# nlesc-dirac/sagecal

Hardware: NVIDIA H100
Metric: baseline_visibilities_per_sec_predict_jacobian (higher is better)
Workload: dtype f64

## Files before the change

sagecal_b200/csrc/internal.cuh:

```cuda
#pragma once
#include <cuda_runtime.h>
#include <stdint.h>
#include <stdio.h>
#include <stdlib.h>

#define DB_CHECK(call)                                                                          \
  do {                                                                                          \
    cudaError_t err__ = (call);                                                                 \
    if (err__ != cudaSuccess) {                                                                 \
      fprintf(stderr, "dirac_b200: CUDA error %s at %s:%d: %s\n", cudaGetErrorName(err__),      \
              __FILE__, __LINE__, cudaGetErrorString(err__));                                   \
      exit(1);          \
    }                                                                                           \
  } while (0)


#define TILE_P 8
#define TILE_Q 32
#define TILE_THREADS (TILE_P * TILE_Q)

struct TileDesc {
  short pb, qb;
};

// ... 250 lines not shown
  const double *mu_dev;
  double mu;
  int lower;
  int N, Nbase;
};

enum { DB_OPT_CP_ROWS = 0, DB_OPT_LINE_DIRECT = 1, DB_OPT_OS_CONSISTENT = 2,
       DB_OPT_RTR_NU_UNJOINED = 3, DB_OPT_ADMM_LM = 4, DB_OPT_SWEEP_RESIDUAL = 5,
       DB_OPT_COUNT = 8 };
int db_opt(int id);
int db_sm_count();
static inline int db_cp_max_slices(int Nbase, int tilesz) {
  const int nbg = (Nbase + 255) / 256;
  int nsl = (db_sm_count() + nbg - 1) / nbg;
  if ((tilesz + 31) / 32 > nsl) nsl = (tilesz + 31) / 32;
  return nsl;
}

extern "C" {
void db_launch_coh_to_planar(const double2 *src, double2 *dst, long long r0, int nr, int M,
                             long long R, cudaStream_t st);
void db_launch_coh_from_planar(const double2 *src, double2 *dst, long long r0, int nr, int M,
                               long long R, cudaStream_t st);
void db_launch_vis_to_planar(const double2 *src, double2 *dst, long long R, cudaStream_t st);
void db_launch_vis_from_planar(const double2 *src, double2 *dst, long long R, cudaStream_t st);
void db_launch_grad_tma(const GradArgs *a, int ntile, cudaStream_t st);
void db_launch_grad_window_tma(const GradArgs *a, int ntile, long long r_lo, long long r_hi,
                               cudaStream_t st);
void db_launch_grad_band_tma(const GradArgs *a, int ntile, int nchan, cudaStream_t st);
int db_cluster_pass_nblocks(int ntile, int nt, int tslice);
enum { DB_CP_LIN = 0, DB_CP_LIN_GRAD = 1, DB_CP_SPLIT = 2, DB_CP_TILE = 3, DB_CP_NONE = 4 };
int db_launch_cluster_pass(const ClusterPassArgs *a, int ntile, cudaStream_t st);
int db_cluster_pass_forms_hidden(int N, int Nbase);
void db_launch_coh_gram(const GramArgs *a, int ntile, int nk, cudaStream_t st);
void db_launch_station_sums(const AssembleArgs *a, int nb, cudaStream_t st);
void db_launch_assemble_tiles(const AssembleArgs *a, int nb, cudaStream_t st);
void db_launch_batch_mu0(const double *Hst, double *mu, int N, double tau, int nb, cudaStream_t st);
void db_launch_copy_add_diag(const double *A0, double *A, int n, double mu, cudaStream_t st);
int db_chol_max_n();
int db_chol_available();
size_t db_chol_ws_doubles(int n);
int db_tri_available(int n);
void db_chol_set_step(const double *pcur, double *pnew, double *sc, double *zero);
void db_launch_tri_solve(const double *L, int n, const double *b, double *x, cudaStream_t st);
void db_launch_tri_solve_ld(const double *L, int ld, int n, const double *b, double *x,
                            cudaStream_t st);
void db_launch_chol_factor_batched(const double *A, int n, const double *mu, double *ws,
                                   long long ws_stride, int *info, int nb, cudaStream_t st);
void db_launch_chol_solve(const double *A, int n, double mu, const double *b, double *x, double *ws,
                          int *info, cudaStream_t st);
int db_bigtri_available(int n);
size_t db_bigtri_ws_doubles(int n);
void db_launch_bigtri_solve(const double *L, int ld, int n, const double *b, double *x, double *ws,
                            unsigned epoch, int invert, cudaStream_t st);
int db_stream_all_nblocks(int Nbase, int tilesz);
void db_launch_predict_tma(const StreamAllArgs *a, cudaStream_t st);
void db_launch_cost_window_tma(const StreamAllArgs *a, cudaStream_t st);
int db_band_nblocks(int Nbase, int tilesz, int nchan);
void db_launch_band_tma(const StreamAllArgs *a, int nchan, cudaStream_t st);
void db_launch_band_tma(const StreamAllArgs *a, int nchan, cudaStream_t st);
unsigned db_launch_line_setup_tma(const StreamAllArgs *a, cudaStream_t st);
void db_launch_line_poly_finish(const double *part, unsigned nparts, double *partials, double *out,
                                unsigned int *counter, cudaStream_t st);
void db_line_setup_shape_reset();
void db_line_setup_shape(int *shape);
}
```

sagecal_b200/csrc/kernels_bigtri.cu:

```cuda
#include "internal.cuh"

#define BT 64
#define BT_THREADS 256
#define BT_PENDING 0x7ff8dead0badbeefull

__device__ __forceinline__ unsigned ld_acquire(const unsigned *p) {
  unsigned v;
  asm volatile("ld.acquire.gpu.u32 %0, [%1];" : "=r"(v) : "l"(p) : "memory");
  return v;
}
__device__ __forceinline__ void st_release(unsigned *p, unsigned v) {
  asm volatile("st.release.gpu.u32 [%0], %1;" ::"l"(p), "r"(v) : "memory");
}

__global__ void __launch_bounds__(BT)
k_bigtri_diag_inv(const double *__restrict__ L, int ld, double *__restrict__ Linv) {
  __shared__ double Ls[BT * BT];
  const int blk = blockIdx.x, c = threadIdx.x;
  const double *src = L + (size_t)(blk * BT) * ld + blk * BT;
  for (int e = threadIdx.x; e < BT * BT; e += BT) {
    const int cc = e / BT, r = e % BT;
    Ls[cc * BT + r] = (r >= cc) ? src[(size_t)cc * ld + r] : 0.0;
  }
  __syncthreads();
  double x[BT];
#pragma unroll
  for (int r = 0; r < BT; r++) x[r] = 0.0;
#pragma unroll
  for (int r = 0; r < BT; r++) {
    double s = (r == c) ? 1.0 : 0.0;
#pragma unroll
    for (int k = 0; k < BT; k++)
      if (k < r) s = fma(-Ls[k * BT + r], x[k], s);
    x[r] = (r >= c) ? s / Ls[r * BT + r] : 0.0;
  }
  double *dst = Linv + (size_t)blk * BT * BT + (size_t)c * BT;
#pragma unroll
  for (int r = 0; r < BT; r++) dst[r] = x[r];
}

struct BigTriArgs {
  const double *L;
  const double *Linv;
  const double *rhs;
  double *out;
  unsigned *flags;
  unsigned epoch;
  int n, ld, nb;
};

template <bool FWD>
__global__ void __launch_bounds__(BT_THREADS)
k_bigtri(BigTriArgs a) {
  extern __shared__ __align__(16) double sm[];
  double *Lc = sm;
  double *Li = Lc + BT * BT;
  double *vec = Li + BT * BT;
  double *part = vec + BT;
  const int tid = threadIdx.x, r = tid & (BT - 1), q = tid >> 6;
  const int me = FWD ? (int)blockIdx.x : a.nb - 1 - (int)blockIdx.x;
  const int nprev = FWD ? me : a.nb - 1 - me;
  {
    const double *inv = a.Linv + (size_t)me * BT * BT;
    for (int e = tid; e < BT * BT; e += BT_THREADS) {
      const int cc = e / BT, rr = e % BT;
      if (FWD) Li[cc * BT + rr] = inv[e];
      else Li[rr * BT + cc] = inv[e];
    }
    if (nprev > 0) {
      const int bi = FWD ? me : me + 1, bk = FWD ? me - 1 : me;
      const double *src = a.L + (size_t)(bk * BT) * a.ld + bi * BT;
      for (int e = tid; e < BT * BT; e += BT_THREADS) {
        const int cc = e / BT, rr = e % BT;
        const double v = src[(size_t)cc * a.ld + rr];
        if (FWD) Lc[cc * BT + rr] = v;
        else Lc[rr * BT + cc] = v;
      }
    }
  }
  double acc = 0.0;
  double nx[16];
  auto fetch = [&](int step) {
    const int other = FWD ? step : a.nb - 1 - step;
    if (FWD) {
      const double *src = a.L + (size_t)(other * BT + 16 * q) * a.ld + me * BT + r;
#pragma unroll
      for (int c = 0; c < 16; c++) nx[c] = __ldcg(src + (size_t)c * a.ld);
    } else {
      const double *src = a.L + (size_t)(me * BT + r) * a.ld + other * BT + 16 * q;
#pragma unroll
      for (int c = 0; c < 16; c++) nx[c] = __ldcg(src + c);
    }
  };
  const int noff = nprev > 0 ? nprev - 1 : 0;
  if (noff > 0) fetch(0);
  __syncthreads();
  for (int step = 0; step < nprev; step++) {
    const int other = FWD ? step : a.nb - 1 - step;
    if (tid < BT) {
      const unsigned long long *src = reinterpret_cast<const unsigned long long *>(a.out) +
                                      (size_t)other * BT + tid;
      unsigned long long bits;
      do {
        asm volatile("ld.relaxed.gpu.u64 %0, [%1];" : "=l"(bits) : "l"(src) : "memory");
      } while (bits == BT_PENDING);
      vec[tid] = __longlong_as_double((long long)bits);
    }
    __syncthreads();
    if (step < noff) {
      double cur[16];
#pragma unroll
      for (int c = 0; c < 16; c++) cur[c] = nx[c];
      if (step + 1 < noff) fetch(step + 1);
#pragma unroll
      for (int c = 0; c < 16; c++) acc = fma(-cur[c], vec[16 * q + c], acc);
    } else {
#pragma unroll
      for (int c = 0; c < 16; c++) acc = fma(-Lc[(16 * q + c) * BT + r], vec[16 * q + c], acc);
    }
    __syncthreads();
  }
  part[q * BT + r] = acc;
  __syncthreads();
  if (tid < BT)
    vec[tid] = a.rhs[(size_t)me * BT + tid] + part[tid] + part[BT + tid] + part[2 * BT + tid] +
               part[3 * BT + tid];
  __syncthreads();
  double s = 0.0;
#pragma unroll
  for (int c = 0; c < 16; c++) s = fma(Li[(16 * q + c) * BT + r], vec[16 * q + c], s);
  __syncthreads();
  part[q * BT + r] = s;
  __syncthreads();
  if (tid < BT) {
    const double v = part[tid] + part[BT + tid] + part[2 * BT + tid] + part[3 * BT + tid];
    asm volatile("st.relaxed.gpu.f64 [%0], %1;" ::"l"(a.out + (size_t)me * BT + tid), "d"(v) : "memory");
  }
}

__global__ void k_bigtri_arm(unsigned long long *y, unsigned long long *x, int n) {
  const int i = blockIdx.x * blockDim.x + threadIdx.x;
  if (i < n) {
    y[i] = BT_PENDING;
    x[i] = BT_PENDING;
  }
}

extern "C" {
int db_bigtri_available(int n) {
  if (getenv("DIRAC_B200_NO_BIGTRI")) return 0;
  return n > 512 && (n % BT) == 0 && n / BT <= db_sm_count();
}
size_t db_bigtri_ws_doubles(int n) { return (size_t)(n / BT) * BT * BT + (size_t)n + (size_t)(n / BT) + 16; }

void db_launch_bigtri_solve(const double *L, int ld, int n, const double *b, double *x, double *ws,
                            unsigned epoch, int invert, cudaStream_t st) {
  const int nb = n / BT;
  double *Linv = ws, *y = ws + (size_t)nb * BT * BT;
  unsigned *flags = reinterpret_cast<unsigned *>(y + n);
  static bool configured = false;
  const size_t smem = sizeof(double) * (2 * BT * BT + BT + 4 * BT);
  if (!configured) {
    DB_CHECK(cudaFuncSetAttribute(k_bigtri<true>, cudaFuncAttributeMaxDynamicSharedMemorySize, (int)smem));
    DB_CHECK(cudaFuncSetAttribute(k_bigtri<false>, cudaFuncAttributeMaxDynamicSharedMemorySize, (int)smem));
    configured = true;
  }
  if (invert) k_bigtri_diag_inv<<<nb, BT, 0, st>>>(L, ld, Linv);
  k_bigtri_arm<<<(n + 255) / 256, 256, 0, st>>>(reinterpret_cast<unsigned long long *>(y),
                                               reinterpret_cast<unsigned long long *>(x), n);
  BigTriArgs a;
  a.L = L; a.Linv = Linv; a.n = n; a.ld = ld; a.nb = nb;
  a.rhs = b; a.out = y; a.flags = flags; a.epoch = 2 * epoch + 1;
  k_bigtri<true><<<nb, BT_THREADS, smem, st>>>(a);
  a.rhs = y; a.out = x; a.flags = flags + nb; a.epoch = 2 * epoch + 2;
  k_bigtri<false><<<nb, BT_THREADS, smem, st>>>(a);
}

int dirac_b200_bigtri_solve(int n, const double *L, const double *b, double *x, int reps, double *us) {
  if (!db_bigtri_available(n)) return -1;
  double *dL, *db, *dx, *ws;
  const size_t nd = db_bigtri_ws_doubles(n);
  DB_CHECK(cudaMalloc((void **)&dL, sizeof(double) * (size_t)n * n));
  DB_CHECK(cudaMalloc((void **)&db, sizeof(double) * n));
  DB_CHECK(cudaMalloc((void **)&dx, sizeof(double) * n));
  DB_CHECK(cudaMalloc((void **)&ws, sizeof(double) * nd));
  DB_CHECK(cudaMemset(ws, 0, sizeof(double) * nd));
  DB_CHECK(cudaMemcpy(dL, L, sizeof(double) * (size_t)n * n, cudaMemcpyHostToDevice));
  DB_CHECK(cudaMemcpy(db, b, sizeof(double) * n, cudaMemcpyHostToDevice));
  unsigned epoch = 0;
  db_launch_bigtri_solve(dL, n, n, db, dx, ws, ++epoch, 1, 0);
  DB_CHECK(cudaDeviceSynchronize());
  DB_CHECK(cudaMemcpy(x, dx, sizeof(double) * n, cudaMemcpyDeviceToHost));
  if (reps > 0 && us) {
    cudaEvent_t e0, e1;
    DB_CHECK(cudaEventCreate(&e0));
    DB_CHECK(cudaEventCreate(&e1));
    DB_CHECK(cudaEventRecord(e0, 0));
    for (int i = 0; i < reps; i++) db_launch_bigtri_solve(dL, n, n, db, dx, ws, ++epoch, 0, 0);
    DB_CHECK(cudaEventRecord(e1, 0));
    DB_CHECK(cudaEventSynchronize(e1));
    float ms = 0.f;
    DB_CHECK(cudaEventElapsedTime(&ms, e0, e1));
    *us = 1e3 * ms / reps;
    cudaEventDestroy(e0);
    cudaEventDestroy(e1);
  }
  DB_CHECK(cudaGetLastError());
  cudaFree(dL); cudaFree(db); cudaFree(dx); cudaFree(ws);
  return 0;
}
}
```

sagecal_b200/csrc/lm.cu:

```cuda
#include <float.h>
#include <math.h>
#include <string.h>
#include <vector>

#include "../../include/dirac_b200.h"
#include "problem.h"

#define CS_CHECK(call)                                                                     \
  do {                                                                                     \
    cusolverStatus_t s__ = (call);                                                         \
    if (s__ != CUSOLVER_STATUS_SUCCESS) {                                                  \
      fprintf(stderr, "dirac_b200: cuSOLVER error %d at %s:%d\n", (int)s__, __FILE__, __LINE__); \
      exit(1);                                                                             \
    }                                                                                      \
  } while (0)
#define CB_CHECK(call)                                                                     \
  do {                                                                                     \
    cublasStatus_t s__ = (call);                                                           \
    if (s__ != CUBLAS_STATUS_SUCCESS) {                                                    \
      fprintf(stderr, "dirac_b200: cuBLAS error %d at %s:%d\n", (int)s__, __FILE__, __LINE__); \
      exit(1);                                                                             \
    }                                                                                      \
  } while (0)

// ... 30 lines not shown
  w.Tsub = dalloc<double>((size_t)d.Nbase * 16);
  w.JTJ0 = dalloc<double>((size_t)n8 * n8);
  w.JTJ = dalloc<double>((size_t)n8 * n8);
  w.JTe = d.scal + 64 + n8;
  w.JTe_new = d.scal + 64 + 2 * n8;
  w.Hst = dalloc<double>((size_t)4 * d.N);
  w.Dp = d.scal + 64;
  w.pnew = dalloc<double>(n8);
  w.plast = dalloc<double>(n8);
  w.pold = dalloc<double>(n8);
  w.devinfo = reinterpret_cast<int *>(d.scal + 64 + 3 * n8);
  w.tau = dalloc<double>(n8);
  w.svdS = w.svdU = w.svdVT = nullptr;
  w.wbuf = w.ebuf = nullptr;
  w.os_eps = w.os_w = nullptr;
  w.HP = w.HQ = nullptr;
  w.JB = w.LB = nullptr;
  w.sys_T = w.sys_p = w.sys_H = nullptr;
  w.pref_slot = (int *)malloc(sizeof(int) * d.M);
  for (int k = 0; k < d.M; k++) w.pref_slot[k] = -1;
  w.jtj0_cur = nullptr;
  w.jtj_spec = nullptr;
  {
    const int nbg = (d.Nbase + 255) / 256;
    const int nsl = db_cp_max_slices(d.Nbase, d.tilesz);
    w.jte_part = dalloc<double>((size_t)nbg * (nsl + 1) * n8);
  }
  DB_CHECK(cudaEventCreateWithFlags(&w.ev_mail, cudaEventDisableTiming));
  DB_CHECK(cudaMallocHost((void **)&w.h_vec, sizeof(double) * (5 * n8 + 4 * d.N + 64)));
  static cusolverDnHandle_t g_cs = nullptr;
  static cublasHandle_t g_cb = nullptr;
  if (!g_cs) {
    CS_CHECK(cusolverDnCreate(&g_cs));
    CB_CHECK(cublasCreate(&g_cb));
  }
  w.cs = g_cs;
  w.cb = g_cb;
  CS_CHECK(cusolverDnSetStream(w.cs, d.stream));
  CB_CHECK(cublasSetStream(w.cb, d.stream));
  int l1 = 0, l2 = 0, l3 = 0;
  CS_CHECK(cusolverDnDpotrf_bufferSize(w.cs, CUBLAS_FILL_MODE_LOWER, n8, w.JTJ, n8, &l1));
  CS_CHECK(cusolverDnDgeqrf_bufferSize(w.cs, n8, n8, w.JTJ, n8, &l2));
  CS_CHECK(cusolverDnDormqr_bufferSize(w.cs, CUBLAS_SIDE_LEFT, CUBLAS_OP_T, n8, 1, n8, w.JTJ, n8,
                                       w.tau, w.Dp, n8, &l3));
  w.lwork = l1 > l2 ? l1 : l2;
  if (l3 > w.lwork) w.lwork = l3;
  int l4 = 0;
  CS_CHECK(cusolverDnDgesvd_bufferSize(w.cs, n8, n8, &l4));
  if (l4 > w.lwork) w.lwork = l4;
  w.own_chol = n8 <= db_chol_max_n() && db_chol_available() && !getenv("DIRAC_B200_CUSOLVER");
  if (w.own_chol && (size_t)w.lwork < db_chol_ws_doubles(n8)) w.lwork = (int)db_chol_ws_doubles(n8);
  w.cswork = dalloc<double>((size_t)w.lwork);
  w.bc = (!w.own_chol && n8 > 1024) ? db_bigchol_create(n8, BC_BLOCK, BC_INV_PANEL, BC_LOOKAHEAD) : nullptr;
  w.bt_ws = nullptr;
  w.bt_epoch = 0;
  if (!w.own_chol && db_bigtri_available(n8)) {
    const size_t nd = db_bigtri_ws_doubles(n8);
    w.bt_ws = dalloc<double>(nd);
    DB_CHECK(cudaMemsetAsync(w.bt_ws, 0, sizeof(double) * nd, d.stream));
  }
  w.dbuf = dalloc<double2>((size_t)4 * d.R);
  w.ready = true;
}

static void robust_init(dirac_b200_problem *pr) {
  LMWork &w = pr->lm;
  if (w.wbuf) return;
  DevProblem &d = pr->d;
  w.wbuf = dalloc<double2>((size_t)4 * d.R);
  w.ebuf = dalloc<double2>((size_t)4 * d.R);
  w.HP = dalloc<double>((size_t)d.N * 20);
  w.HQ = dalloc<double>((size_t)d.N * 20);
}

static void os_init(dirac_b200_problem *pr) {
  robust_init(pr);
  LMWork &w = pr->lm;
  if (w.os_eps) return;
  w.os_eps = dalloc<double2>((size_t)4 * pr->d.R);
  w.os_w = dalloc<double2>((size_t)4 * pr->d.R);
}

void db_lm_free(dirac_b200_problem *pr) {
  LMWork &w = pr->lm;
  if (!w.ready) return;
  db_free(w.T); db_free(w.Tsub); db_free(w.JTJ0); db_free(w.JTJ);
  db_free(w.Hst); db_free(w.pnew); db_free(w.plast); db_free(w.pold); db_free(w.jte_part);
  db_free(w.tau); db_free(w.cswork); db_free(w.dbuf);
  if (w.bt_ws) db_free(w.bt_ws);
  db_bigchol_destroy(w.bc);
  if (w.svdS) { db_free(w.svdS); db_free(w.svdU); db_free(w.svdVT); }
  if (w.wbuf) { db_free(w.wbuf); db_free(w.ebuf); db_free(w.HP); db_free(w.HQ); }
  if (w.os_eps) { db_free(w.os_eps); db_free(w.os_w); }
  if (w.LB) {
    if (w.JB) db_free(w.JB);
    db_free(w.LB); db_free(w.HB); db_free(w.mu_dev); db_free(w.binfo_dev);
    db_free(w.LBptr_dev); db_free(w.blist_dev); db_free(w.btix_dev); db_free(w.bpoff_dev);
    cudaFreeHost(w.h_mu); cudaFreeHost(w.h_binfo);
  }
  free(w.pref_slot);
  cudaEventDestroy(w.ev_mail);
  cudaFreeHost(w.h_vec);
  free(w.T_valid);
  w.ready = false;
}

static int pick_tslice(const DevProblem &d, int nt) {
  int target_ctas = db_sm_count();
  int slices = (target_ctas + d.ntile - 1) / d.ntile;
  if (slices < 1) slices = 1;
  int ts = (nt + slices - 1) / slices;
  if (ts < 2) ts = 2;
  if (ts > nt) ts = nt;
// ... 96 lines not shown
  WeightedJtjArgs a;
  a.coh_k = d.coh + (size_t)k * 4 * d.R;
  a.wt = wt; a.flag = d.flag; a.pblk = pblk_dev; a.tiles = d.tiles; a.JTJ = JTJ; a.HP = w.HP;
  a.HQ = w.HQ; a.R = d.R; a.N = d.N; a.Nbase = d.Nbase; a.t_begin = t0; a.t_end = t1;
  a.tslice = pick_tslice(d, t1 - t0);
  db_prof_begin(6, (double)(t1 - t0) * d.Nbase * 129.0 + 8.0 * 64.0 * d.N * d.N, d.stream);
  db_launch_weighted_jtj(&a, d.ntile, d.stream);
  db_prof_end(d.stream);
  db_count_launch(2);
}

void db_chunk_range(const DevProblem &d, int k, int ck, int *t0, int *t1);
static void chunk_range(const DevProblem &d, int k, int ck, int *t0, int *t1) {
  db_chunk_range(d, k, ck, t0, t1);
}
void db_chunk_range(const DevProblem &d, int k, int ck, int *t0, int *t1) {
  int nchunk = d.h_clus[k].nchunk;
  int tilechunk = (d.tilesz + nchunk - 1) / nchunk;
  int a = ck * tilechunk;
  int b = a + tilechunk;
  if (a > d.tilesz) a = d.tilesz;
  if (b > d.tilesz) b = d.tilesz;
  *t0 = a;
  *t1 = b;
}

static int enqueue_solve(dirac_b200_problem *pr, double mu, int linsolv, double eps1) {
  DevProblem &d = pr->d;
  LMWork &w = pr->lm;
  const int n = w.n8;
  int *hinfo = (int *)(w.h_vec + 4 * n + 4 * d.N);
  hinfo[0] = hinfo[1] = 0;
  if (linsolv == 0 && w.own_chol) {
    db_prof_begin(5, 0.0, d.stream);
    db_launch_chol_solve(w.jtj0_cur ? w.jtj0_cur : w.JTJ0, n, mu, w.JTe, w.Dp, w.cswork, w.devinfo,
                         d.stream);
    db_prof_end(d.stream);
    db_count_launch(1);
    w.step_fused = w.step_armed;
    return 1;
  }
  if (linsolv == 0 && w.sys_T) {
    AssembleArgs a = assemble_args(d, w.sys_T, w.sys_p, const_cast<double *>(w.sys_H));
    a.JTJ = w.JTJ;
    a.mu = mu;
    a.lower = 1;
    assemble_tiles(pr, a, 1);
  } else {
    db_prof_begin(4, 16.0 * n * n, d.stream);
    db_launch_copy_add_diag(w.jtj0_cur ? w.jtj0_cur : w.JTJ0, w.JTJ, n, mu, d.stream);
    db_prof_end(d.stream);
    db_count_launch(1);
  }
  DB_CHECK(cudaMemcpyAsync(w.Dp, w.JTe, sizeof(double) * n, cudaMemcpyDeviceToDevice, d.stream));
  db_prof_begin(5, 0.0, d.stream);
  if (linsolv == 0) {
    CS_CHECK(cusolverDnDpotrf(w.cs, CUBLAS_FILL_MODE_LOWER, n, w.JTJ, n, w.cswork, w.lwork,
                              w.devinfo));
    if (w.bt_ws) {
      DB_CHECK(cudaMemsetAsync(w.devinfo + 1, 0, sizeof(int), d.stream));
      db_launch_bigtri_solve(w.JTJ, n, n, w.JTe, w.Dp, w.bt_ws, ++w.bt_epoch, 1, d.stream);
      db_count_launch(4);
    } else {
      CS_CHECK(cusolverDnDpotrs(w.cs, CUBLAS_FILL_MODE_LOWER, n, 1, w.JTJ, n, w.Dp, n,
                                w.devinfo + 1));
      db_count_launch(2);
    }
  } else if (linsolv == 1) {
    CS_CHECK(cusolverDnDgeqrf(w.cs, n, n, w.JTJ, n, w.tau, w.cswork, w.lwork, w.devinfo));
    CS_CHECK(cusolverDnDormqr(w.cs, CUBLAS_SIDE_LEFT, CUBLAS_OP_T, n, 1, n, w.JTJ, n, w.tau, w.Dp,
                              n, w.cswork, w.lwork, w.devinfo + 1));
    const double one = 1.0;
    CB_CHECK(cublasDtrsm(w.cb, CUBLAS_SIDE_LEFT, CUBLAS_FILL_MODE_UPPER, CUBLAS_OP_N,
                         CUBLAS_DIAG_NON_UNIT, n, 1, &one, w.JTJ, n, w.Dp, n));
    db_count_launch(3);
  } else {
    if (!w.svdS) {
      w.svdS = dalloc<double>(n);
      w.svdU = dalloc<double>((size_t)n * n);
      w.svdVT = dalloc<double>((size_t)n * n);
    }
    CS_CHECK(cusolverDnDgesvd(w.cs, 'A', 'A', n, n, w.JTJ, n, w.svdS, w.svdU, n, w.svdVT, n,
                              w.cswork, w.lwork, nullptr, w.devinfo));
    db_count_launch(1);
    double *hS = (double *)malloc(sizeof(double) * n);
    double *hb = (double *)malloc(sizeof(double) * n);
    const double one = 1.0, zero = 0.0;
    CB_CHECK(cublasDgemv(w.cb, CUBLAS_OP_T, n, n, &one, w.svdU, n, w.JTe, 1, &zero, w.Dp, 1));
    DB_CHECK(cudaMemcpyAsync(hS, w.svdS, sizeof(double) * n, cudaMemcpyDeviceToHost, d.stream));
    DB_CHECK(cudaMemcpyAsync(hb, w.Dp, sizeof(double) * n, cudaMemcpyDeviceToHost, d.stream));
    db_stream_sync(d.stream);
    for (int i = 0; i < n; i++) hb[i] = (hS[i] > eps1) ? hb[i] / hS[i] : 0.0;
    DB_CHECK(cudaMemcpyAsync(w.pnew, hb, sizeof(double) * n, cudaMemcpyHostToDevice, d.stream));
    CB_CHECK(cublasDgemv(w.cb, CUBLAS_OP_T, n, n, &one, w.svdVT, n, w.pnew, 1, &zero, w.Dp, 1));
    db_prof_end(d.stream);
    DB_CHECK(cudaMemcpyAsync(w.h_vec + 2 * n, w.Dp, sizeof(double) * n, cudaMemcpyDeviceToHost,
                             d.stream));
    db_stream_sync(d.stream);
    free(hS);
    free(hb);
    db_count_launch(2);
    return 1;
  }
  db_prof_end(d.stream);
  (void)hinfo;
  return 1;
}

static double nrm2sq(const double *v, int n) {
  double s = 0.0;
  for (int i = 0; i < n; i++) s += v[i] * v[i];
  return s;
}

void db_prefactor_sweep(dirac_b200_problem *pr, double tau) {
// ... 335 lines not shown
          db_launch_extract_diag(w.JTJ0, w.JTe_new, n, d.stream);
          db_count_launch(1);
          DB_CHECK(cudaMemcpyAsync(hsc, w.JTe_new, sizeof(double) * n, cudaMemcpyDeviceToHost,
                                   d.stream));
        } else {
          DB_CHECK(cudaMemcpyAsync(hH, w.Hst, sizeof(double) * 4 * d.N, cudaMemcpyDeviceToHost,
                                   d.stream));
        }
      }
      if (need_mx || os) db_stream_sync(d.stream);
      if (need_mx) {
        if (wt || os_misaligned) {
          for (int i = 0; i < n; i++)
            if (fabs(hsc[i]) > fabs(mx)) mx = hsc[i];
        } else {
          for (int s = 0; s < d.N; s++) {
            if (fabs(hH[4 * s]) > fabs(mx)) mx = hH[4 * s];
            if (fabs(hH[4 * s + 1]) > fabs(mx)) mx = hH[4 * s + 1];
          }
        }
      }
      double p_L2 = 0.0;
      if (!pending_entry) {
        jacTe_inf = 0.0;
        for (int i = 0; i < n; i++) {
          double a = fabs(hjte[i]);
          if (a > jacTe_inf) jacTe_inf = a;
        }
        p_L2 = nrm2sq(hp, n);
        if (jacTe_inf <= eps1) {
          Dp_L2 = 0.0;
          stop = 1;
          if (!os) kiter_adjust = 1;
          break;
        }
      }
      if (kiter == 0) mu = prefac ? w.h_mu[slot] : tau * (mx + half_rho);
      bool use_factor = prefac;
      while (1) {
        int issolved;
        bool skip_info = false;
        w.step_fused = false;
        w.step_armed = w.own_chol && linsolv == 0;
        if (w.step_armed)
          db_chol_set_step(pblk_dev, w.pnew, d.scal + 8, os ? nullptr : w.JTe_new);
        if (use_factor) {
          use_factor = false;
          db_prof_begin(5, 0.0, d.stream);
          if (w.own_chol && db_tri_available(n)) {
            skip_info = true;
            db_launch_tri_solve_ld(w.LB + (size_t)slot * w.lb_stride, w.lb_ld, n, w.JTe, w.Dp,
                                   d.stream);
            w.step_fused = w.step_armed;
          } else {
            DB_CHECK(cudaMemsetAsync(w.devinfo, 0, 2 * sizeof(int), d.stream));
            if (w.bt_ws) {
              db_launch_bigtri_solve(w.LB + (size_t)slot * w.lb_stride, n, n, w.JTe, w.Dp, w.bt_ws,
                                     ++w.bt_epoch, 1, d.stream);
            } else {
              DB_CHECK(cudaMemcpyAsync(w.Dp, w.JTe, sizeof(double) * n, cudaMemcpyDeviceToDevice,
                                       d.stream));
              CS_CHECK(cusolverDnDpotrs(w.cs, CUBLAS_FILL_MODE_LOWER, n, 1,
                                        w.LB + (size_t)slot * w.lb_stride, n, w.Dp, n, w.devinfo + 1));
            }
          }
          db_prof_end(d.stream);
          db_count_launch(1);
          issolved = (w.h_binfo[slot * w.binfo_step] == 0) ? 1 : 0;
        } else {
          issolved = enqueue_solve(pr, mu + half_rho, linsolv, eps1);
        }
        if (w.step_armed) db_chol_set_step(nullptr, nullptr, nullptr, nullptr);
        if (!w.step_fused)
          db_launch_lm_step(pblk_dev, w.Dp, w.JTe, w.pnew, d.scal + 8, os ? nullptr : w.JTe_new, n,
                            d.stream);
        if (hidden_from) {
          const bool last = kiter == itmax - 1;
          db_cluster_pass(pr, k, w.pnew, hidden_from, last ? w.dbuf : nullptr, 1, last ? 1 : 0,
                          last ? nullptr : w.JTe_new, 1, t0, t1, nullptr, 1.0, true, w.pold,
                          true);
        } else {
          db_cluster_pass(pr, k, w.pnew, w.dbuf, nullptr, 1, 0, os ? nullptr : w.JTe_new, 1, t0, t1,
                          wt, 1.0, true);
        }
        if (aug)
          db_launch_lm_aug_rhs(w.JTe_new, w.pnew, aug->y_dev, aug->bz_dev, aug->rho, n, d.stream);
        if (!w.step_fused) db_count_launch(1);
        int *hinfo = (int *)(w.h_vec + 4 * n + 4 * d.N);
        DB_CHECK(cudaMemcpyAsync(d.h_scal, d.scal, sizeof(double) * (64 + 3 * n + 2),
                                 cudaMemcpyDeviceToHost, d.stream));
        double *spec_buf = nullptr;
        if (w.own_chol && linsolv == 0 && !wt && !os && kiter + 1 < itmax && w.T_valid[tix]) {
          const double *cur = w.jtj0_cur ? w.jtj0_cur : w.JTJ0;
          spec_buf = (cur == w.JTJ0) ? w.JTJ : w.JTJ0;
          DB_CHECK(cudaEventRecord(w.ev_mail, d.stream));
          assemble(pr, Tfull, w.pnew, spec_buf);
          db_event_sync(w.ev_mail);
        } else {
          db_stream_sync(d.stream);
        }
        {
          const double *hm = d.h_scal + 64;
          memcpy(hDp, hm, sizeof(double) * n);
          hsc[n] = d.h_scal[8];
          hsc[n + 1] = d.h_scal[9];
          hsc[n + 2] = d.h_scal[1];
          if (!os) memcpy(hjte_new, hm + (w.JTe_new - w.Dp), sizeof(double) * n);
          if (pending_entry) memcpy(hjte, hm + (w.JTe - w.Dp), sizeof(double) * n);
          memcpy(hinfo, hm + 3 * n, 2 * sizeof(int));
          if (skip_info) hinfo[0] = hinfo[1] = 0;
        }
        if (pending_entry) {
          pending_entry = false;
          p_eL2 = init_p_eL2 = d.h_scal[2];
          if (!isfinite(p_eL2)) {
            stop = 7;
            kiter_adjust = 1;
// ... 582 lines not shown
```

sagecal_b200/csrc/problem.h:

```cpp
#pragma once
#include <cusolverDn.h>
#include <cublas_v2.h>

#include <vector>

#include "../../include/dirac_b200.h"
#include "internal.cuh"

struct BigChol;
BigChol *db_bigchol_create(int n, int nbk, bool inv_panel, bool lookahead);
enum { BC_BLOCK = 256 };
static const bool BC_INV_PANEL = true, BC_LOOKAHEAD = true;
void db_bigchol_destroy(BigChol *bc);
void db_bigchol_bind_batch(BigChol *bc, double *A0, long long stride, int maxb);
void db_bigchol_factor_batch(BigChol *bc, int nb, int *info, int info_step, cudaStream_t st);

struct LMWork {
  bool ready;
  int n8;
  double *T;
  unsigned char *T_valid;
  double *Tsub;
  double *JTJ0, *JTJ;
  double *JTe, *JTe_new;
  double *Hst;
  double *Dp;
  double *pnew;
  double *h_vec;
  int *devinfo;
  double *cswork;
  int lwork;
  bool own_chol;
  double *bt_ws;
  unsigned bt_epoch;
  BigChol *bc;
  double *jte_part;
  bool step_armed, step_fused;
  double *jtj_spec;
  cudaEvent_t ev_mail;
  double *tau;
  double *svdS, *svdU, *svdVT;
  cusolverDnHandle_t cs;
  cublasHandle_t cb;
  double2 *dbuf;
  double2 *wbuf;
  double2 *ebuf;
  double2 *os_eps, *os_w;
  double *HP, *HQ;
  double *plast;
  double *pold;
  double *JB, *LB;
  size_t lb_stride;
  int lb_ld, binfo_step;
  double *HB;
  double *mu_dev;
  double *h_mu;
  int *binfo_dev, *h_binfo;
  double **LBptr_dev;
  int *blist_dev, *btix_dev, *bpoff_dev;
  int *pref_slot;
  const double *jtj0_cur;
  const double *sys_T, *sys_p, *sys_H;
};

struct dirac_b200_problem {
  DevProblem d;
  double *partials;
  int npartials;
  double2 *res;
  double2 *vis_stage;
  double *g;
  LMWork lm;
  int own_stream;
  int rank, world;
  void (*allreduce)(void *dev, long long count, void *stream, void *user);
  void *comm_user;
  int m_global;
  int k_global0;
  double beta;
  const double *aug_y_host, *aug_bz_host, *aug_rho;
  double *aug_dev;
  double2 *pm;
  double *xb;
  double *pp_start;
  double2 *E0, *E1, *E2;
  double *poly_part;
  struct RtrWork *rtr;
// ... 116 lines not shown
```

Measured before the change: 7.204 billion.

## Fuse forward/backward big triangular solves into one persistent kernel with cp.async ring

Replaces the separate forward and backward block-triangular solve kernels with a prep kernel and a single kernel. The prep kernel inverts the diagonal blocks, precomputes the products of those inverses with the neighbouring off-diagonal blocks, and arms the pending flags. The solve kernel streams off-diagonal tiles through a multi-stage cp.async ring and does both sweeps with dataflow polling between blocks. This removes a launch and the flag arming kernel, drops a device copy and memset in the LM step, and puts diagonal inversion on every call. A benchmark script for the solve sequence is also added.

```diff
diff --git a/profiles/bigtri_solve.py b/profiles/bigtri_solve.py
--- /dev/null
+++ b/profiles/bigtri_solve.py
@@ -0,0 +1,53 @@
+import argparse
+import ctypes as C
+import json
+import os
+import sys
+
+import numpy as np
+
+ROOT = os.path.dirname(os.path.dirname(os.path.abspath(__file__)))
+sys.path.insert(0, ROOT)
+sys.path.insert(0, os.path.dirname(os.path.abspath(__file__)))
+from sagecal_b200 import lib as blib
+from minibatch_stage import card
+
+
+def spd(n, seed):
+    g = np.random.default_rng(seed).standard_normal((n, n))
+    return g @ g.T / n + 0.5 * np.eye(n)
+
+
+def main():
+    import scipy.linalg as sla
+    ap = argparse.ArgumentParser()
+    ap.add_argument("--n", type=int, default=4096)
+    ap.add_argument("--nfac", type=int, default=2)
+    ap.add_argument("--reps", type=int, default=400)
+    ap.add_argument("--lib", default=blib.LIB_PATH)
+    args = ap.parse_args()
+    n, nfac = args.n, args.nfac
+    L = blib.DiracB200(os.path.abspath(args.lib)).lib
+    f = L.dirac_b200_bigtri_sequence
+    f.restype = C.c_int
+    f.argtypes = [C.c_int, C.c_int, C.c_void_p, C.c_int, C.c_void_p, C.c_void_p, C.c_int, C.c_void_p]
+    mats = [spd(n, 10 + i) for i in range(nfac)]
+    A = np.stack([np.asfortranarray(m) for m in mats]).copy()
+    b = np.random.default_rng(3).standard_normal((nfac, n))
+    x = np.zeros((nfac, n))
+    us = np.zeros(2)
+    rc = f(n, nfac, A.ctypes.data, nfac, b.ctypes.data, x.ctypes.data, args.reps, us.ctypes.data)
+    if rc != 0:
+        raise SystemExit("dirac_b200_bigtri_sequence returned %d" % rc)
+    rel = max(float(np.max(np.abs(x[i] - want)) / np.max(np.abs(want)))
+              for i, want in enumerate(sla.cho_solve(sla.cho_factor(m, lower=True), b[i]) for i, m in enumerate(mats)))
+    rep = {"lib": os.path.relpath(os.path.abspath(args.lib), ROOT), "n": n, "nfac": nfac, "reps": args.reps}
+    rep["card"], rep["power_limit_and_max_sm_clock"] = card()
+    rep["us_per_substitution_pair"] = round(float(us[0]), 1)
+    rep["us_per_dpotrf"] = round(float(us[1]), 1)
+    rep["max_rel_err_vs_scipy"] = rel
+    print(json.dumps(rep))
+
+
+if __name__ == "__main__":
+    main()
diff --git a/sagecal_b200/csrc/internal.cuh b/sagecal_b200/csrc/internal.cuh
--- a/sagecal_b200/csrc/internal.cuh
+++ b/sagecal_b200/csrc/internal.cuh
@@ -326,7 +326,7 @@
 int db_bigtri_available(int n);
 size_t db_bigtri_ws_doubles(int n);
 void db_launch_bigtri_solve(const double *L, int ld, int n, const double *b, double *x, double *ws,
-                            unsigned epoch, int invert, cudaStream_t st);
+                            int *status, cudaStream_t st);
 int db_stream_all_nblocks(int Nbase, int tilesz);
 void db_launch_predict_tma(const StreamAllArgs *a, cudaStream_t st);
 void db_launch_cost_window_tma(const StreamAllArgs *a, cudaStream_t st);
diff --git a/sagecal_b200/csrc/kernels_bigtri.cu b/sagecal_b200/csrc/kernels_bigtri.cu
--- a/sagecal_b200/csrc/kernels_bigtri.cu
+++ b/sagecal_b200/csrc/kernels_bigtri.cu
@@ -1,194 +1,252 @@
 #include "internal.cuh"
+#include <cusolverDn.h>
+#include <vector>
 
 #define BT 64
 #define BT_THREADS 256
+#define BT_STAGES 4
 #define BT_PENDING 0x7ff8dead0badbeefull
 
-__device__ __forceinline__ unsigned ld_acquire(const unsigned *p) {
-  unsigned v;
-  asm volatile("ld.acquire.gpu.u32 %0, [%1];" : "=r"(v) : "l"(p) : "memory");
-  return v;
-}
-__device__ __forceinline__ void st_release(unsigned *p, unsigned v) {
-  asm volatile("st.release.gpu.u32 [%0], %1;" ::"l"(p), "r"(v) : "memory");
-}
-
-__global__ void __launch_bounds__(BT)
-k_bigtri_diag_inv(const double *__restrict__ L, int ld, double *__restrict__ Linv) {
-  __shared__ double Ls[BT * BT];
-  const int blk = blockIdx.x, c = threadIdx.x;
-  const double *src = L + (size_t)(blk * BT) * ld + blk * BT;
-  for (int e = threadIdx.x; e < BT * BT; e += BT) {
-    const int cc = e / BT, r = e % BT;
-    Ls[cc * BT + r] = (r >= cc) ? src[(size_t)cc * ld + r] : 0.0;
-  }
-  __syncthreads();
-  double x[BT];
-#pragma unroll
-  for (int r = 0; r < BT; r++) x[r] = 0.0;
-#pragma unroll
-  for (int r = 0; r < BT; r++) {
-    double s = (r == c) ? 1.0 : 0.0;
-#pragma unroll
-    for (int k = 0; k < BT; k++)
-      if (k < r) s = fma(-Ls[k * BT + r], x[k], s);
-    x[r] = (r >= c) ? s / Ls[r * BT + r] : 0.0;
-  }
-  double *dst = Linv + (size_t)blk * BT * BT + (size_t)c * BT;
-#pragma unroll
-  for (int r = 0; r < BT; r++) dst[r] = x[r];
+__host__ __device__ __forceinline__ int bt_idx(int row, int col) {
+  return (col >> 2) * BT_THREADS + row * 4 + (col & 3);
+}
+
+__global__ void __launch_bounds__(BT_THREADS)
+k_bigtri_prep(const double *__restrict__ L, int ld, int nb, double *__restrict__ Linv,
+              double *__restrict__ M, double *__restrict__ N, unsigned long long *y,
+              unsigned long long *x, int *status) {
+  extern __shared__ double sp[];
+  double *Ls = sp, *Ic = Ls + BT * 65, *Ys = Ic + BT * 65;
+  double *Ir = Ls;
+  const int b = blockIdx.x, tid = threadIdx.x, r = tid >> 2, q = tid & 3;
+  if (tid < BT) {
+    y[b * BT + tid] = BT_PENDING;
+    x[b * BT + tid] = BT_PENDING;
+  }
+  if (b == 0 && tid == 0 && status) *status = 0;
+  const double *Lbb = L + (size_t)(b * BT) * ld + b * BT;
+  for (int e = tid; e < BT * BT; e += BT_THREADS) Ls[(e >> 6) * 65 + (e & 63)] = Lbb[(size_t)(e >> 6) * ld + (e & 63)];
+  __syncthreads();
+  double z[BT];
+  if (tid < BT) {
+#pragma unroll
+    for (int k = 0; k < BT; k++) z[k] = (k == tid) ? 1.0 : 0.0;
+#pragma unroll
+    for (int k = 0; k < BT; k++) {
+      const double zk = z[k] / Ls[k * 65 + k];
+      z[k] = zk;
+#pragma unroll
+      for (int rr = k + 1; rr < BT; rr++) z[rr] = fma(-Ls[k * 65 + rr], zk, z[rr]);
+    }
+  }
+  __syncthreads();
+  if (tid < BT) {
+    double *dst = Linv + (size_t)b * BT * BT;
+#pragma unroll
+    for (int rr = 0; rr < BT; rr++) {
+      Ic[tid * 65 + rr] = z[rr];
+      Ir[rr * 65 + tid] = z[rr];
+      dst[bt_idx(rr, tid)] = z[rr];
+    }
+  }
+  auto product = [&](const double *Xs, double *out) {
+    double p[16];
+#pragma unroll
+    for (int c = 0; c < 16; c++) p[c] = 0.0;
+#pragma unroll 4
+    for (int k = 0; k < BT; k++) {
+      const double xr = Xs[k * 65 + r];
+#pragma unroll
+      for (int c = 0; c < 16; c++) p[c] = fma(xr, Ys[(4 * c + q) * 65 + k], p[c]);
+    }
+#pragma unroll
+    for (int c = 0; c < 16; c++) out[c * BT_THREADS + tid] = p[c];
+  };
+  if (b > 0) {
+    const double *src = L + (size_t)((b - 1) * BT) * ld + b * BT;
+    for (int e = tid; e < BT * BT; e += BT_THREADS) Ys[(e >> 6) * 65 + (e & 63)] = src[(size_t)(e >> 6) * ld + (e & 63)];
+    __syncthreads();
+    product(Ic, M + (size_t)b * BT * BT);
+  }
+  if (b < nb - 1) {
+    __syncthreads();
+    const double *src = L + (size_t)(b * BT) * ld + (b + 1) * BT;
+    for (int e = tid; e < BT * BT; e += BT_THREADS) Ys[(e & 63) * 65 + (e >> 6)] = src[(size_t)(e >> 6) * ld + (e & 63)];
+    __syncthreads();
+    product(Ir, N + (size_t)b * BT * BT);
+  }
 }
 
 struct BigTriArgs {
-  const double *L;
-  const double *Linv;
-  const double *rhs;
-  double *out;
-  unsigned *flags;
-  unsigned epoch;
-  int n, ld, nb;
+  const double *L, *Linv, *M, *N;
+  const double *b;
+  double *y, *x;
+  int ld, nb;
 };
 
-template <bool FWD>
-__global__ void __launch_bounds__(BT_THREADS)
+__device__ __forceinline__ void cp_async8(double *dst, const double *src) {
+  asm volatile("cp.async.ca.shared.global [%0], [%1], 8;" ::"r"((unsigned)__cvta_generic_to_shared(dst)),
+               "l"(src)
+               : "memory");
+}
+
+__device__ __forceinline__ double quad_sum(double v) {
+  v += __shfl_xor_sync(0xffffffffu, v, 1);
+  return v + __shfl_xor_sync(0xffffffffu, v, 2);
+}
+
+__device__ __forceinline__ void await_block(const double *slot, double *vw, int lane) {
+  const unsigned long long *p = reinterpret_cast<const unsigned long long *>(slot);
+  unsigned long long u, v;
+  do {
+    asm volatile("ld.relaxed.gpu.u64 %0, [%1];" : "=l"(u) : "l"(p + lane) : "memory");
+    asm volatile("ld.relaxed.gpu.u64 %0, [%1];" : "=l"(v) : "l"(p + lane + 32) : "memory");
+  } while (u == BT_PENDING || v == BT_PENDING);
+  __syncwarp();
+  vw[lane] = __longlong_as_double((long long)u);
+  vw[lane + 32] = __longlong_as_double((long long)v);
+  __syncwarp();
+}
+
+__global__ void __launch_bounds__(BT_THREADS, 1)
 k_bigtri(BigTriArgs a) {
   extern __shared__ __align__(16) double sm[];
-  double *Lc = sm;
-  double *Li = Lc + BT * BT;
-  double *vec = Li + BT * BT;
-  double *part = vec + BT;
-  const int tid = threadIdx.x, r = tid & (BT - 1), q = tid >> 6;
-  const int me = FWD ? (int)blockIdx.x : a.nb - 1 - (int)blockIdx.x;
-  const int nprev = FWD ? me : a.nb - 1 - me;
-  {
-    const double *inv = a.Linv + (size_t)me * BT * BT;
-    for (int e = tid; e < BT * BT; e += BT_THREADS) {
-      const int cc = e / BT, rr = e % BT;
-      if (FWD) Li[cc * BT + rr] = inv[e];
-      else Li[rr * BT + cc] = inv[e];
-    }
-    if (nprev > 0) {
-      const int bi = FWD ? me : me + 1, bk = FWD ? me - 1 : me;
-      const double *src = a.L + (size_t)(bk * BT) * a.ld + bi * BT;
-      for (int e = tid; e < BT * BT; e += BT_THREADS) {
-        const int cc = e / BT, rr = e % BT;
-        const double v = src[(size_t)cc * a.ld + rr];
-        if (FWD) Lc[cc * BT + rr] = v;
-        else Lc[rr * BT + cc] = v;
+  double *ring = sm;
+  double *LiF = ring + BT_STAGES * 16 * BT_THREADS;
+  double *LiB = LiF + 16 * BT_THREADS;
+  double *vec = LiB + 16 * BT_THREADS;
+  double *sv = vec + 8 * BT;
+  const int tid = threadIdx.x, lane = tid & 31, r = tid >> 2, q = tid & 3;
+  const int me = blockIdx.x, nb = a.nb;
+  double *vw = vec + (tid >> 5) * BT;
+  const int nf = me > 1 ? me - 1 : 0;
+  const int nbw = me < nb - 2 ? nb - 2 - me : 0;
+  const int ntot = nf + nbw;
+  const double *Lf = a.L + (size_t)q * a.ld + me * BT + r;
+  const double *Lb = a.L + (size_t)(me * BT + r) * a.ld + q;
+  auto issue = [&](int blk) {
+    if (blk < ntot) {
+      double *dst = ring + (blk % BT_STAGES) * 16 * BT_THREADS + tid;
+      if (blk < nf) {
+        const double *src = Lf + (size_t)(blk * BT) * a.ld;
+#pragma unroll
+        for (int c = 0; c < 16; c++) cp_async8(dst + c * BT_THREADS, src + (size_t)(4 * c) * a.ld);
+      } else {
+        const double *src = Lb + (nb - 1 - (blk - nf)) * BT;
+#pragma unroll
+        for (int c = 0; c < 16; c++) cp_async8(dst + c * BT_THREADS, src + 4 * c);
       }
     }
-  }
-  double acc = 0.0;
-  double nx[16];
-  auto fetch = [&](int step) {
-    const int other = FWD ? step : a.nb - 1 - step;
-    if (FWD) {
-      const double *src = a.L + (size_t)(other * BT + 16 * q) * a.ld + me * BT + r;
-#pragma unroll
-      for (int c = 0; c < 16; c++) nx[c] = __ldcg(src + (size_t)c * a.ld);
-    } else {
-      const double *src = a.L + (size_t)(me * BT + r) * a.ld + other * BT + 16 * q;
-#pragma unroll
-      for (int c = 0; c < 16; c++) nx[c] = __ldcg(src + c);
-    }
+    asm volatile("cp.async.commit_group;" ::: "memory");
   };
-  const int noff = nprev > 0 ? nprev - 1 : 0;
-  if (noff > 0) fetch(0);
-  __syncthreads();
-  for (int step = 0; step < nprev; step++) {
-    const int other = FWD ? step : a.nb - 1 - step;
-    if (tid < BT) {
-      const unsigned long long *src = reinterpret_cast<const unsigned long long *>(a.out) +
-                                      (size_t)other * BT + tid;
-      unsigned long long bits;
-      do {
-        asm volatile("ld.relaxed.gpu.u64 %0, [%1];" : "=l"(bits) : "l"(src) : "memory");
-      } while (bits == BT_PENDING);
-      vec[tid] = __longlong_as_double((long long)bits);
-    }
-    __syncthreads();
-    if (step < noff) {
-      double cur[16];
-#pragma unroll
-      for (int c = 0; c < 16; c++) cur[c] = nx[c];
-      if (step + 1 < noff) fetch(step + 1);
-#pragma unroll
-      for (int c = 0; c < 16; c++) acc = fma(-cur[c], vec[16 * q + c], acc);
-    } else {
-#pragma unroll
-      for (int c = 0; c < 16; c++) acc = fma(-Lc[(16 * q + c) * BT + r], vec[16 * q + c], acc);
-    }
-    __syncthreads();
-  }
-  part[q * BT + r] = acc;
-  __syncthreads();
-  if (tid < BT)
-    vec[tid] = a.rhs[(size_t)me * BT + tid] + part[tid] + part[BT + tid] + part[2 * BT + tid] +
-               part[3 * BT + tid];
-  __syncthreads();
-  double s = 0.0;
-#pragma unroll
-  for (int c = 0; c < 16; c++) s = fma(Li[(16 * q + c) * BT + r], vec[16 * q + c], s);
-  __syncthreads();
-  part[q * BT + r] = s;
-  __syncthreads();
-  if (tid < BT) {
-    const double v = part[tid] + part[BT + tid] + part[2 * BT + tid] + part[3 * BT + tid];
-    asm volatile("st.relaxed.gpu.f64 [%0], %1;" ::"l"(a.out + (size_t)me * BT + tid), "d"(v) : "memory");
-  }
-}
-
-__global__ void k_bigtri_arm(unsigned long long *y, unsigned long long *x, int n) {
-  const int i = blockIdx.x * blockDim.x + threadIdx.x;
-  if (i < n) {
-    y[i] = BT_PENDING;
-    x[i] = BT_PENDING;
-  }
-}
+  auto consume = [&](int blk, double acc) {
+    asm volatile("cp.async.wait_group %0;" ::"n"(BT_STAGES - 2) : "memory");
+    issue(blk + BT_STAGES - 1);
+    const double *src = ring + (blk % BT_STAGES) * 16 * BT_THREADS + tid;
+#pragma unroll
+    for (int c = 0; c < 16; c++) acc = fma(-src[c * BT_THREADS], vw[4 * c + q], acc);
+    return acc;
+  };
+  for (int s = 0; s < BT_STAGES - 1; s++) issue(s);
+  const size_t off = (size_t)me * BT * BT;
+  double Mr[16], Nr[16];
+#pragma unroll
+  for (int c = 0; c < 16; c++) {
+    Mr[c] = me > 0 ? __ldg(a.M + off + c * BT_THREADS + tid) : 0.0;
+    Nr[c] = me < nb - 1 ? __ldg(a.N + off + c * BT_THREADS + tid) : 0.0;
+    LiF[c * BT_THREADS + tid] = __ldg(a.Linv + off + c * BT_THREADS + tid);
+    LiB[c * BT_THREADS + tid] = __ldg(a.Linv + off + bt_idx(4 * c + q, r));
+  }
+  double acc = q == 0 ? a.b[me * BT + r] : 0.0;
+  for (int k = 0; k < nf; k++) {
+    await_block(a.y + (size_t)k * BT, vw, lane);
+    acc = consume(k, acc);
+  }
+  acc = quad_sum(acc);
+  if (q == 0) sv[r] = acc;
+  __syncthreads();
+  double u = 0.0;
+#pragma unroll
+  for (int c = 0; c < 16; c++) u = fma(LiF[c * BT_THREADS + tid], sv[4 * c + q], u);
+  u = quad_sum(u);
+  if (me > 0) {
+    await_block(a.y + (size_t)(me - 1) * BT, vw, lane);
+    double p0 = 0.0, p1 = 0.0;
+#pragma unroll
+    for (int c = 0; c < 16; c += 2) {
+      p0 = fma(Mr[c], vw[4 * c + q], p0);
+      p1 = fma(Mr[c + 1], vw[4 * c + 4 + q], p1);
+    }
+    u -= quad_sum(p0 + p1);
+  }
+  const double yr = u;
+  if (q == 0) asm volatile("st.relaxed.gpu.f64 [%0], %1;" ::"l"(a.y + (size_t)me * BT + r), "d"(yr) : "memory");
+  acc = q == 0 ? yr : 0.0;
+  for (int t = 0; t < nbw; t++) {
+    await_block(a.x + (size_t)(nb - 1 - t) * BT, vw, lane);
+    acc = consume(nf + t, acc);
+  }
+  acc = quad_sum(acc);
+  __syncthreads();
+  if (q == 0) sv[r] = acc;
+  __syncthreads();
+  u = 0.0;
+#pragma unroll
+  for (int c = 0; c < 16; c++) u = fma(LiB[c * BT_THREADS + tid], sv[4 * c + q], u);
+  u = quad_sum(u);
+  if (me < nb - 1) {
+    await_block(a.x + (size_t)(me + 1) * BT, vw, lane);
+    double p0 = 0.0, p1 = 0.0;
+#pragma unroll
+    for (int c = 0; c < 16; c += 2) {
+      p0 = fma(Nr[c], vw[4 * c + q], p0);
+      p1 = fma(Nr[c + 1], vw[4 * c + 4 + q], p1);
+    }
+    u -= quad_sum(p0 + p1);
+  }
+  if (q == 0) asm volatile("st.relaxed.gpu.f64 [%0], %1;" ::"l"(a.x + (size_t)me * BT + r), "d"(u) : "memory");
+}
+
+static const size_t bt_prep_smem = sizeof(double) * 3 * BT * 65;
+static const size_t bt_smem = sizeof(double) * ((BT_STAGES + 2) * 16 * BT_THREADS + 8 * BT + BT);
 
 extern "C" {
 int db_bigtri_available(int n) {
   if (getenv("DIRAC_B200_NO_BIGTRI")) return 0;
   return n > 512 && (n % BT) == 0 && n / BT <= db_sm_count();
 }
-size_t db_bigtri_ws_doubles(int n) { return (size_t)(n / BT) * BT * BT + (size_t)n + (size_t)(n / BT) + 16; }
+size_t db_bigtri_ws_doubles(int n) { return (size_t)3 * (n / BT) * BT * BT + (size_t)n; }
 
 void db_launch_bigtri_solve(const double *L, int ld, int n, const double *b, double *x, double *ws,
-                            unsigned epoch, int invert, cudaStream_t st) {
+                            int *status, cudaStream_t st) {
   const int nb = n / BT;
-  double *Linv = ws, *y = ws + (size_t)nb * BT * BT;
-  unsigned *flags = reinterpret_cast<unsigned *>(y + n);
+  const size_t blk = (size_t)nb * BT * BT;
+  BigTriArgs a;
+  a.L = L; a.ld = ld; a.nb = nb; a.b = b; a.x = x;
+  a.Linv = ws; a.M = ws + blk; a.N = ws + 2 * blk; a.y = ws + 3 * blk;
   static bool configured = false;
-  const size_t smem = sizeof(double) * (2 * BT * BT + BT + 4 * BT);
   if (!configured) {
-    DB_CHECK(cudaFuncSetAttribute(k_bigtri<true>, cudaFuncAttributeMaxDynamicSharedMemorySize, (int)smem));
-    DB_CHECK(cudaFuncSetAttribute(k_bigtri<false>, cudaFuncAttributeMaxDynamicSharedMemorySize, (int)smem));
+    DB_CHECK(cudaFuncSetAttribute(k_bigtri_prep, cudaFuncAttributeMaxDynamicSharedMemorySize, (int)bt_prep_smem));
+    DB_CHECK(cudaFuncSetAttribute(k_bigtri, cudaFuncAttributeMaxDynamicSharedMemorySize, (int)bt_smem));
     configured = true;
   }
-  if (invert) k_bigtri_diag_inv<<<nb, BT, 0, st>>>(L, ld, Linv);
-  k_bigtri_arm<<<(n + 255) / 256, 256, 0, st>>>(reinterpret_cast<unsigned long long *>(y),
-                                               reinterpret_cast<unsigned long long *>(x), n);
-  BigTriArgs a;
-  a.L = L; a.Linv = Linv; a.n = n; a.ld = ld; a.nb = nb;
-  a.rhs = b; a.out = y; a.flags = flags; a.epoch = 2 * epoch + 1;
-  k_bigtri<true><<<nb, BT_THREADS, smem, st>>>(a);
-  a.rhs = y; a.out = x; a.flags = flags + nb; a.epoch = 2 * epoch + 2;
-  k_bigtri<false><<<nb, BT_THREADS, smem, st>>>(a);
+  k_bigtri_prep<<<nb, BT_THREADS, bt_prep_smem, st>>>(L, ld, nb, ws, ws + blk, ws + 2 * blk,
+                                                      reinterpret_cast<unsigned long long *>(a.y),
+                                                      reinterpret_cast<unsigned long long *>(x), status);
+  void *args[] = {&a};
+  DB_CHECK(cudaLaunchCooperativeKernel((const void *)k_bigtri, dim3(nb), dim3(BT_THREADS), args, bt_smem, st));
 }
 
 int dirac_b200_bigtri_solve(int n, const double *L, const double *b, double *x, int reps, double *us) {
   if (!db_bigtri_available(n)) return -1;
   double *dL, *db, *dx, *ws;
-  const size_t nd = db_bigtri_ws_doubles(n);
   DB_CHECK(cudaMalloc((void **)&dL, sizeof(double) * (size_t)n * n));
   DB_CHECK(cudaMalloc((void **)&db, sizeof(double) * n));
   DB_CHECK(cudaMalloc((void **)&dx, sizeof(double) * n));
-  DB_CHECK(cudaMalloc((void **)&ws, sizeof(double) * nd));
-  DB_CHECK(cudaMemset(ws, 0, sizeof(double) * nd));
+  DB_CHECK(cudaMalloc((void **)&ws, sizeof(double) * db_bigtri_ws_doubles(n)));
   DB_CHECK(cudaMemcpy(dL, L, sizeof(double) * (size_t)n * n, cudaMemcpyHostToDevice));
   DB_CHECK(cudaMemcpy(db, b, sizeof(double) * n, cudaMemcpyHostToDevice));
-  unsigned epoch = 0;
-  db_launch_bigtri_solve(dL, n, n, db, dx, ws, ++epoch, 1, 0);
+  db_launch_bigtri_solve(dL, n, n, db, dx, ws, nullptr, 0);
   DB_CHECK(cudaDeviceSynchronize());
   DB_CHECK(cudaMemcpy(x, dx, sizeof(double) * n, cudaMemcpyDeviceToHost));
   if (reps > 0 && us) {
@@ -196,7 +254,7 @@
     DB_CHECK(cudaEventCreate(&e0));
     DB_CHECK(cudaEventCreate(&e1));
     DB_CHECK(cudaEventRecord(e0, 0));
-    for (int i = 0; i < reps; i++) db_launch_bigtri_solve(dL, n, n, db, dx, ws, ++epoch, 0, 0);
+    for (int i = 0; i < reps; i++) db_launch_bigtri_solve(dL, n, n, db, dx, ws, nullptr, 0);
     DB_CHECK(cudaEventRecord(e1, 0));
     DB_CHECK(cudaEventSynchronize(e1));
     float ms = 0.f;
@@ -209,4 +267,72 @@
   cudaFree(dL); cudaFree(db); cudaFree(dx); cudaFree(ws);
   return 0;
 }
-}
+
+int dirac_b200_bigtri_sequence(int n, int nfac, const double *A, int nsolve, const double *b,
+                               double *x, int reps, double *us) {
+  if (!db_bigtri_available(n) || nfac < 1 || nsolve < 1) return -1;
+  const size_t nn = (size_t)n * n;
+  double *dA, *dcopy, *db, *dx, *dans, *ws, *work;
+  int *info, lwork = 0;
+  cusolverDnHandle_t cs;
+  if (cusolverDnCreate(&cs) != CUSOLVER_STATUS_SUCCESS) return -1;
+  DB_CHECK(cudaMalloc((void **)&dA, sizeof(double) * nn * nfac));
+  DB_CHECK(cudaMalloc((void **)&dcopy, sizeof(double) * nn));
+  DB_CHECK(cudaMalloc((void **)&db, sizeof(double) * (size_t)n * nsolve));
+  DB_CHECK(cudaMalloc((void **)&dans, sizeof(double) * (size_t)n * nsolve));
+  DB_CHECK(cudaMalloc((void **)&dx, sizeof(double) * n));
+  DB_CHECK(cudaMalloc((void **)&ws, sizeof(double) * db_bigtri_ws_doubles(n)));
+  DB_CHECK(cudaMalloc((void **)&info, sizeof(int) * (nfac + 1)));
+  DB_CHECK(cudaMemcpy(dA, A, sizeof(double) * nn * nfac, cudaMemcpyHostToDevice));
+  DB_CHECK(cudaMemcpy(dcopy, dA, sizeof(double) * nn, cudaMemcpyDeviceToDevice));
+  DB_CHECK(cudaMemcpy(db, b, sizeof(double) * (size_t)n * nsolve, cudaMemcpyHostToDevice));
+  cusolverDnDpotrf_bufferSize(cs, CUBLAS_FILL_MODE_LOWER, n, dA, n, &lwork);
+  DB_CHECK(cudaMalloc((void **)&work, sizeof(double) * (lwork + 1)));
+  int rc = 0;
+  std::vector<int> hinfo(nfac);
+  for (int f = 0; f < nfac; f++)
+    cusolverDnDpotrf(cs, CUBLAS_FILL_MODE_LOWER, n, dA + nn * f, n, work, lwork, info + f);
+  DB_CHECK(cudaMemcpy(hinfo.data(), info, sizeof(int) * nfac, cudaMemcpyDeviceToHost));
+  for (int f = 0; f < nfac; f++)
+    if (hinfo[f]) rc = -2;
+  if (rc == 0) {
+    for (int s = 0; s < nsolve; s++) {
+      db_launch_bigtri_solve(dA + nn * (s % nfac), n, n, db + (size_t)n * s, dx, ws, info + nfac, 0);
+      DB_CHECK(cudaMemcpyAsync(dans + (size_t)n * s, dx, sizeof(double) * n, cudaMemcpyDeviceToDevice, 0));
+    }
+    DB_CHECK(cudaDeviceSynchronize());
+    DB_CHECK(cudaMemcpy(x, dans, sizeof(double) * (size_t)n * nsolve, cudaMemcpyDeviceToHost));
+  }
+  if (rc == 0 && reps > 0 && us) {
+    cudaEvent_t e0, e1;
+    DB_CHECK(cudaEventCreate(&e0));
+    DB_CHECK(cudaEventCreate(&e1));
+    float ms = 0.f, t = 0.f;
+    for (int i = 0; i < 3 + nfac; i++) db_launch_bigtri_solve(dA + nn * (i % nfac), n, n, db, dx, ws, info + nfac, 0);
+    DB_CHECK(cudaEventRecord(e0, 0));
+    for (int i = 0; i < reps; i++) db_launch_bigtri_solve(dA + nn * (i % nfac), n, n, db, dx, ws, info + nfac, 0);
+    DB_CHECK(cudaEventRecord(e1, 0));
+    DB_CHECK(cudaEventSynchronize(e1));
+    DB_CHECK(cudaEventElapsedTime(&ms, e0, e1));
+    us[0] = 1e3 * ms / reps;
+    ms = 0.f;
+    for (int i = 0; i < reps + 1; i++) {
+      DB_CHECK(cudaMemcpyAsync(dA, dcopy, sizeof(double) * nn, cudaMemcpyDeviceToDevice, 0));
+      DB_CHECK(cudaEventRecord(e0, 0));
+      cusolverDnDpotrf(cs, CUBLAS_FILL_MODE_LOWER, n, dA, n, work, lwork, info);
+      DB_CHECK(cudaEventRecord(e1, 0));
+      DB_CHECK(cudaEventSynchronize(e1));
+      DB_CHECK(cudaEventElapsedTime(&t, e0, e1));
+      if (i > 0) ms += t;
+    }
+    us[1] = 1e3 * ms / reps;
+    cudaEventDestroy(e0);
+    cudaEventDestroy(e1);
+  }
+  DB_CHECK(cudaGetLastError());
+  cudaFree(dA); cudaFree(dcopy); cudaFree(db); cudaFree(dans); cudaFree(dx); cudaFree(ws); cudaFree(info);
+  cudaFree(work);
+  cusolverDnDestroy(cs);
+  return rc;
+}
+}
diff --git a/sagecal_b200/csrc/lm.cu b/sagecal_b200/csrc/lm.cu
--- a/sagecal_b200/csrc/lm.cu
+++ b/sagecal_b200/csrc/lm.cu
@@ -106,13 +106,7 @@
   if (w.own_chol && (size_t)w.lwork < db_chol_ws_doubles(n8)) w.lwork = (int)db_chol_ws_doubles(n8);
   w.cswork = dalloc<double>((size_t)w.lwork);
   w.bc = (!w.own_chol && n8 > 1024) ? db_bigchol_create(n8, BC_BLOCK, BC_INV_PANEL, BC_LOOKAHEAD) : nullptr;
-  w.bt_ws = nullptr;
-  w.bt_epoch = 0;
-  if (!w.own_chol && db_bigtri_available(n8)) {
-    const size_t nd = db_bigtri_ws_doubles(n8);
-    w.bt_ws = dalloc<double>(nd);
-    DB_CHECK(cudaMemsetAsync(w.bt_ws, 0, sizeof(double) * nd, d.stream));
-  }
+  w.bt_ws = (!w.own_chol && db_bigtri_available(n8)) ? dalloc<double>(db_bigtri_ws_doubles(n8)) : nullptr;
   w.dbuf = dalloc<double2>((size_t)4 * d.R);
   w.ready = true;
 }
@@ -315,15 +309,15 @@
     db_prof_end(d.stream);
     db_count_launch(1);
   }
-  DB_CHECK(cudaMemcpyAsync(w.Dp, w.JTe, sizeof(double) * n, cudaMemcpyDeviceToDevice, d.stream));
+  if (linsolv != 0 || !w.bt_ws)
+    DB_CHECK(cudaMemcpyAsync(w.Dp, w.JTe, sizeof(double) * n, cudaMemcpyDeviceToDevice, d.stream));
   db_prof_begin(5, 0.0, d.stream);
   if (linsolv == 0) {
     CS_CHECK(cusolverDnDpotrf(w.cs, CUBLAS_FILL_MODE_LOWER, n, w.JTJ, n, w.cswork, w.lwork,
                               w.devinfo));
     if (w.bt_ws) {
-      DB_CHECK(cudaMemsetAsync(w.devinfo + 1, 0, sizeof(int), d.stream));
-      db_launch_bigtri_solve(w.JTJ, n, n, w.JTe, w.Dp, w.bt_ws, ++w.bt_epoch, 1, d.stream);
-      db_count_launch(4);
+      db_launch_bigtri_solve(w.JTJ, n, n, w.JTe, w.Dp, w.bt_ws, w.devinfo + 1, d.stream);
+      db_count_launch(2);
     } else {
       CS_CHECK(cusolverDnDpotrs(w.cs, CUBLAS_FILL_MODE_LOWER, n, 1, w.JTJ, n, w.Dp, n,
                                 w.devinfo + 1));
@@ -765,17 +759,16 @@
             db_launch_tri_solve_ld(w.LB + (size_t)slot * w.lb_stride, w.lb_ld, n, w.JTe, w.Dp,
                                    d.stream);
             w.step_fused = w.step_armed;
+          } else if (w.bt_ws) {
+            skip_info = true;
+            db_launch_bigtri_solve(w.LB + (size_t)slot * w.lb_stride, n, n, w.JTe, w.Dp, w.bt_ws,
+                                   nullptr, d.stream);
           } else {
             DB_CHECK(cudaMemsetAsync(w.devinfo, 0, 2 * sizeof(int), d.stream));
-            if (w.bt_ws) {
-              db_launch_bigtri_solve(w.LB + (size_t)slot * w.lb_stride, n, n, w.JTe, w.Dp, w.bt_ws,
-                                     ++w.bt_epoch, 1, d.stream);
-            } else {
-              DB_CHECK(cudaMemcpyAsync(w.Dp, w.JTe, sizeof(double) * n, cudaMemcpyDeviceToDevice,
-                                       d.stream));
-              CS_CHECK(cusolverDnDpotrs(w.cs, CUBLAS_FILL_MODE_LOWER, n, 1,
-                                        w.LB + (size_t)slot * w.lb_stride, n, w.Dp, n, w.devinfo + 1));
-            }
+            DB_CHECK(cudaMemcpyAsync(w.Dp, w.JTe, sizeof(double) * n, cudaMemcpyDeviceToDevice,
+                                     d.stream));
+            CS_CHECK(cusolverDnDpotrs(w.cs, CUBLAS_FILL_MODE_LOWER, n, 1,
+                                      w.LB + (size_t)slot * w.lb_stride, n, w.Dp, n, w.devinfo + 1));
           }
           db_prof_end(d.stream);
           db_count_launch(1);
diff --git a/sagecal_b200/csrc/problem.h b/sagecal_b200/csrc/problem.h
--- a/sagecal_b200/csrc/problem.h
+++ b/sagecal_b200/csrc/problem.h
@@ -32,7 +32,6 @@
   int lwork;
   bool own_chol;
   double *bt_ws;
-  unsigned bt_epoch;
   BigChol *bc;
   double *jte_part;
   bool step_armed, step_fused;
```

New measurement: 7.595 billion (median of 6 runs). 1.05x the previous value.
